# IONIQ6000/av1-base

Hardware: AMD Instinct MI355X
Metric: encoded frames/sec at CQ=30 (1080p intra-only) (higher is better)
Workload: dtype i32; 1 GPU; 1920x1080 60-frame all-key-frame synthclip v1 chunk per GPU, 10-bit 4:2:0, CQ=30 (base_q_idx 120), 32x32 blocks, all 13 intra candidates, 64x64 tiles, adaptive CDFs, CDEF on; frames_per_chunk=60, chunks_per_gpu=1, parallelism=chunk-per-gpu x1

## Files before the change

av1-base_amd/csrc/av1mi_dev.h:

```cpp
#ifndef AV1MI_DEV_H
#define AV1MI_DEV_H
#include <stdint.h>
#include <stddef.h>
#ifdef __HIPCC__
#define AV1MI_HD __host__ __device__
#else
#define AV1MI_HD
#endif

#define AV1MI_QM_4X4 0
#define AV1MI_QM_8X8 16
#define AV1MI_QM_16X16 80
#define AV1MI_QM_32X32 336
#define AV1MI_QM_PLANE 1360

struct Av1miQmEntry { uint32_t q, recip; };

struct Av1miChunkRecord {
  unsigned long long n_symbols;
  uint32_t max_tile_symbols;
  int overflow;
};
static_assert(sizeof(Av1miChunkRecord) == 16, "the frame offsets follow the head, 8-byte aligned");

// ... 197 lines not shown
    GLOBALMV = NEWMV + 6 * 3,
    REFMV = GLOBALMV + 2 * 3,
    DRL = REFMV + 6 * 3,
    SINGLE_REF = DRL + 3 * 3,
    INTER_TX1 = SINGLE_REF + 18 * 3,
    INTER_TX2 = INTER_TX1 + 2 * 17,
    INTER_TX3 = INTER_TX2 + 13,
    MV_JOINT = INTER_TX3 + 4 * 3,
    MV_COMP = MV_JOINT + 5,
    MVC_CLASS = 0, MVC_CLASS0_FP = 12, MVC_FP = 22, MVC_SIGN = 27, MVC_CLASS0_HP = 30, MVC_HP = 33, MVC_CLASS0 = 36, MVC_BITS = 39,
    MVC_SIZE = 69,
    TOTAL = MV_COMP + 2 * MVC_SIZE
  };
};

#endif
```

av1-base_amd/csrc/av1mi_host.cpp:

```cpp
#include <hip/hip_runtime.h>
#include <errno.h>
#include <math.h>
#include <stdarg.h>
#include <stdio.h>
#include <stdlib.h>
#include <string.h>
#include <unistd.h>

#include <algorithm>
#include <atomic>
#include <cstddef>
#include <mutex>
#include <string>
#include <thread>
#include <vector>

#include "../../include/av1mi.h"
#include "av1_tables.h"
#include "av1mi_dev.h"
#include "av1mi_launch.h"
#include "lr_fit_rule.h"
#include "wiener_fit_rule.h"
#include "deblock_pieces.h"
#include "aq_rule.h"
// ... 403 lines not shown
  unsigned long long *d_lrsse = nullptr;
  Av1miLrFit fit = {};
  uint8_t *d_fit = nullptr, *h_fit = nullptr;
  Av1miLrWfit wfit = {};
  uint8_t *d_wfit = nullptr, *h_wfit = nullptr;
  unsigned long long *d_cdef_err = nullptr;
  int8_t *d_cdef_idx = nullptr;
  uint8_t *d_cdef_sel = nullptr;
  unsigned long long *d_lf_err = nullptr;
  uint8_t *d_lf_sel = nullptr;
  uint8_t *h_lf = nullptr;
  uint8_t *h_out = nullptr;
  uint8_t *h_hdr = nullptr; uint16_t *h_cdf = nullptr; Av1miDevParams *h_params = nullptr;
  size_t hdr_bytes = 0;
  int cdf_qidx = -1;
  int params_on_device = 0;
  Av1miChunkRecord *h_record = nullptr; unsigned long long *h_sse = nullptr;
  size_t out_cap = 0, me64_bytes = 0, h_out_cap = 0;
  std::vector<std::pair<void *, bool>> owned;
};

template <class T>
hipError_t ws_alloc(Workspace &w, T *&p, size_t bytes, bool host = false) {
  for (auto b = w.owned.begin(); p && b != w.owned.end(); ++b)
    if (b->first == (void *)p) { (void)(b->second ? hipHostFree(p) : hipFree(p)); w.owned.erase(b); break; }
  void *v = nullptr;
  const hipError_t e = host ? hipHostMalloc(&v, bytes, hipHostMallocDefault) : hipMalloc(&v, bytes);
  if (e == hipSuccess) w.owned.emplace_back(v, host);
  p = (T *)v;
  return e;
// ... 64 lines not shown
                    w.scale == c->cap_scale && w.res.tile_sb == r.tile_sb;
  const int bps = p.bit_depth > 8 ? 2 : 1;
  const size_t frame_bytes = (size_t)r.cw * r.ch * 3 / 2 * bps;
  const size_t nsb = (size_t)r.sb_cols * r.sb_rows, ntile = (size_t)r.tile_cols * r.tile_rows, nb8 = (size_t)(r.cw / 8) * (r.ch / 8);
  if (!same) {
    free_workspace(c);
    const size_t nf = n_frames, slot = (size_t)tile_slot_bytes(r, c->cap_scale);
    for (void **b : { &w.d_src, &w.d_rec, &w.d_fin }) HIPCHK(c, ws_alloc(w, *b, nf * frame_bytes));
    HIPCHK(c, ws_alloc(w, w.d_levels, nf * nsb * AV1MI_SB_LEVELS * sizeof(int16_t)));
    HIPCHK(c, ws_alloc(w, w.d_blk, nf * nb8 * sizeof(Av1miBlkInfo)));
    HIPCHK(c, hipMemsetAsync(w.d_blk, 0, nf * nb8 * sizeof(Av1miBlkInfo), c->stream));
    HIPCHK(c, ws_alloc(w, w.d_slots, nf * ntile * slot * 2));
    w.out_cap = nf * (ntile * (slot + 4) + 256);
    HIPCHK(c, ws_alloc(w, w.d_out, w.out_cap));
    HIPCHK(c, ws_alloc(w, w.d_hdr, 256 + nf * 512));
    HIPCHK(c, ws_alloc(w, w.d_cdf, Av1miCdfLayout::TOTAL * sizeof(uint16_t)));
    HIPCHK(c, ws_alloc(w, w.d_params, AV1MI_AQ_SLOTS * sizeof(Av1miDevParams)));
    for (uint32_t **b : { &w.d_tile_bytes, &w.d_tile_off, &w.d_sym, &w.d_combos }) HIPCHK(c, ws_alloc(w, *b, nf * nsb * 4));
    HIPCHK(c, ws_alloc(w, w.d_streams, nf * ntile * (size_t)tile_stream_cap(r, c->cap_scale) * 4));
    for (uint32_t **b : { &w.d_frame_size, &w.d_payload }) HIPCHK(c, ws_alloc(w, *b, nf * 4));
    HIPCHK(c, ws_alloc(w, w.d_record, sizeof(Av1miChunkRecord) + (nf + 1) * 8));
    HIPCHK(c, ws_alloc(w, w.d_sse, nf * 3 * 8));
    {
      auto up = [](size_t n) { return (n + 255) & ~(size_t)255; };
      const size_t b_hdr = up(256 + nf * 512), b_cdf = up(Av1miCdfLayout::TOTAL * sizeof(uint16_t)), b_par = up(AV1MI_AQ_SLOTS * sizeof(Av1miDevParams)),
                   b_rec = up(sizeof(Av1miChunkRecord) + (nf + 1) * 8), b_sse = up(nf * 3 * 8);
      uint8_t *h = nullptr;
      HIPCHK(c, ws_alloc(w, h, b_hdr + b_cdf + b_par + b_rec + b_sse, true));
      w.h_hdr = h; h += b_hdr;
      w.h_cdf = reinterpret_cast<uint16_t *>(h); h += b_cdf;
      w.h_params = reinterpret_cast<Av1miDevParams *>(h); h += b_par;
      w.h_record = reinterpret_cast<Av1miChunkRecord *>(h); h += b_rec;
      w.h_sse = reinterpret_cast<unsigned long long *>(h);
    }
    HIPCHK(c, ws_alloc(w, w.d_me, nf * nb8 * 8));
    w.cap_frames = n_frames; w.scale = c->cap_scale;
  }
  const size_t nf = w.cap_frames;
  if (r.padded && !w.d_stage) HIPCHK(c, ws_alloc(w, w.d_stage, caller_bytes(r, nf)));
  if (p.partition_search && !w.d_part) HIPCHK(c, ws_alloc(w, w.d_part, nf * nsb * sizeof(uint32_t)));
// ... 463 lines not shown
  if (seq.size() > 256 || fh.size() > (size_t)P.hdr_slot_bytes || fhi.size() > (size_t)P.hdr_slot_bytes) { set_err(c, "internal: header larger than its slot"); return AV1MI_E_OVERFLOW; }
  std::vector<uint8_t> blob(seq.size() + (size_t)n_frames * P.hdr_slot_bytes, 0);
  memcpy(blob.data(), seq.data(), seq.size());
  for (uint32_t f = 0; f < n_frames; f++) {
    const bool inter = av1mi_frame_is_inter(P, (int)f);
    std::vector<uint8_t> &h = inter ? fhi : fh;
    if (r.p.film_grain && f) h = make_frame_header(r, nullptr, f, inter);
    memcpy(blob.data() + seq.size() + (size_t)f * P.hdr_slot_bytes, h.data(), h.size());
  }
  if (w.hdr_bytes != blob.size() || memcmp(w.h_hdr, blob.data(), blob.size())) {
    w.hdr_bytes = 0;
    memcpy(w.h_hdr, blob.data(), blob.size());
    HIPCHK(c, hipMemcpyAsync(w.d_hdr, w.h_hdr, blob.size(), hipMemcpyHostToDevice, s));
  }
  w.hdr_bytes = P.cdef_search || P.lf_search ? 0 : blob.size();
  if (w.cdf_qidx != r.qidx) {
    w.cdf_qidx = -1;
    const std::vector<uint16_t> cdf = make_cdf_blob(r.qidx);
    memcpy(w.h_cdf, cdf.data(), cdf.size() * 2);
    HIPCHK(c, hipMemcpyAsync(w.d_cdf, w.h_cdf, cdf.size() * 2, hipMemcpyHostToDevice, s));
    w.cdf_qidx = r.qidx;
  }
  {
    const int n_par = P.aq_map ? AV1MI_AQ_SLOTS : 1;
    std::vector<Av1miDevParams> par((size_t)n_par, P);
    for (int sl = 1; sl < n_par; sl++) {
      Av1miDevParams &Q = par[(size_t)sl];
      set_quant_steps(Q, quant_steps(av1mi_aq_slot_qindex(sl, r.qidx), P.bit_depth));
      if (P.qm_tab) Q.qm_tab = P.qm_tab + (size_t)sl * 2 * AV1MI_QM_PLANE;
    }
    const size_t bytes = (size_t)n_par * sizeof(P);
    if (w.params_on_device < n_par || memcmp(w.h_params, par.data(), bytes)) {
      w.params_on_device = 0;
      memcpy(w.h_params, par.data(), bytes);
      HIPCHK(c, hipMemcpyAsync(w.d_params, w.h_params, bytes, hipMemcpyHostToDevice, s));
      w.params_on_device = n_par;
// ... 264 lines not shown
```

av1-base_amd/csrc/entropy_kernel.hip:

```cpp
#include <hip/hip_runtime.h>
#include <cstdlib>
#include "av1mi_dev.h"
#include "av1mi_launch.h"

namespace {

typedef Av1miCdfLayout CL;

#define ENT_RESOLVED(fl6, fh6, ns) (0x80000000u | ((uint32_t)(fl6) << 14) | ((uint32_t)(fh6) << 4) | (uint32_t)(ns))
#define ENT_NARROW(slot, sym) (((uint32_t)(slot) << 2) | (uint32_t)(sym))
#define ENT_LITERAL(bit) ((bit) ? ENT_RESOLVED(256, 0, 0) : ENT_RESOLVED(512, 256, 1))
#define SLOTS_PER_COMBO 63
#define MAX_COMBOS 2

__shared__ uint16_t g_cdf_narrow[CL::INTRA_TOTAL - CL::COEFF_BASE + 64];
__shared__ uint16_t g_full_list[5 * 64];
__shared__ uint16_t g_cdf_inter[CL::TOTAL - CL::INTER_BASE + 64];
struct InterLds {
  int stk_row[10], stk_col[10], stk_w[10];
  uint8_t newmv[256];
};
__shared__ InterLds g_inter;
struct CC {
  enum {
    LEAD = CL::TX_SET1,
    TXSET = LEAD,
    TXB_SKIP = TXSET + 13 * 8,
    EOB = TXB_SKIP + 2 * 13 * 3,
    EOB_EXTRA = EOB + 2 * 12,
    DC_SIGN = EOB_EXTRA + 2 * 9 * 3,
    COEFF_BASE_EOB = DC_SIGN + 18,
    USE_WIENER = COEFF_BASE_EOB + 2 * 16, RESTORE_SW = USE_WIENER + 3, CFL_SIGN = RESTORE_SW + 4, CFL_ALPHA = CFL_SIGN + 9,
    DELTA_Q = CFL_ALPHA + 6 * 17,
    TOTAL = DELTA_Q + 5
  };
};
static_assert(CL::COEFF_BASE - CL::USE_WIENER == CC::TOTAL - CC::USE_WIENER, "the trailing tables are copied as one piece");
__shared__ uint16_t g_cdfw_full[CL::COEFF_BASE + 18];
__shared__ uint16_t g_cdfw_compact[CC::TOTAL + 18];
struct SymLds {
  alignas(16) int16_t lv[32 * 32];
  uint8_t left_lvl[3][16], left_dc[3][16];
};
__shared__ SymLds g_sym;
#define S (&g_sym)
template <int TSB>
struct TileLds {
  Av1miBlkInfo info[64 * TSB * TSB];
  uint8_t above_lvl[3][16 * TSB], above_dc[3][16 * TSB];
};
__shared__ TileLds<1> g_tile1;
__shared__ TileLds<2> g_tile2;
template <int TSB> struct TileSel;
template <> struct TileSel<1> { static __device__ __forceinline__ TileLds<1> &get() { return g_tile1; } };
template <> struct TileSel<2> { static __device__ __forceinline__ TileLds<2> &get() { return g_tile2; } };
#define TI (TileSel<TSB>::get())
#define TW (8 * TSB)

struct Sym {
  uint16_t *cdf;
  uint32_t *out;
  int pos;
  int cap;
  int combo0, combo1;
};

__device__ __forceinline__ int uni(int v) { return __builtin_amdgcn_readfirstlane(v); }
__device__ __forceinline__ int iabs(int v) { return v < 0 ? -v : v; }
__device__ __forceinline__ int imin(int a, int b) { return a < b ? a : b; }
__device__ __forceinline__ int imax(int a, int b) { return a > b ? a : b; }
__device__ __forceinline__ int floor_log2(unsigned v) { return 31 - __builtin_clz(v); }

__device__ __forceinline__ void emit1(Sym &y, int lane, uint32_t ent) {
  if (lane == 0 && y.pos < y.cap) y.out[y.pos] = ent;
  y.pos++;
}

template <int ARR = 0>
__device__ __forceinline__ void sym_wide(Sym &y, int lane, int adapt, int s, int off, int n) {
  s = uni(s); off = uni(off) - (ARR ? CL::INTER_BASE : 0); n = uni(n);
  const int v = ARR ? g_cdf_inter[off + (lane < 17 ? lane : 16)] : y.cdf[off + (lane < 17 ? lane : 16)];
  const uint32_t fl = s > 0 ? (uint32_t)__builtin_amdgcn_readlane(v, s - 1) : 32768u;
  const uint32_t fh = (uint32_t)__builtin_amdgcn_readlane(v, s);
  if (adapt) {
    const int cntr = __builtin_amdgcn_readlane(v, n);
    const int rate = 3 + (cntr > 15) + (cntr > 31) + (n > 3 ? 2 : 1);
    int nv = lane < s ? v + ((32768 - v) >> rate) : v - (v >> rate);
    nv = lane == n ? cntr + (cntr < 32) : nv;
    if (lane <= n) { if (ARR) g_cdf_inter[off + lane] = (uint16_t)nv; else y.cdf[off + lane] = (uint16_t)nv; }
  }
// ... 74 lines not shown
__device__ __forceinline__ void sym_coeffs(Sym &y, const int lane, const int adapt, const TileGeo &tg, int plane, int log2n, int x4,
                                           int y4, int eob, int ymode, int is_inter, const int16_t *lv_global) {
  const int idtx = ymode >> 8;
  ymode &= 255;
  const int ptype = plane > 0;
  const int txs = log2n - 2;
  const int w4 = (1 << log2n) >> 2;
  const int bwl = log2n > 5 ? 5 : log2n;
  const int n = 1 << bwl;
  const int max_x4 = plane ? tg.max_x4_c : tg.max_x4_y, max_y4 = plane ? tg.max_y4_c : tg.max_y4_y;
  const int aoff = (plane ? tg.tox >> 3 : tg.tox >> 2);
#define a_lvl (TI.above_lvl[plane] + aoff)
#define a_dc (TI.above_dc[plane] + aoff)
#define l_lvl S->left_lvl[plane]
#define l_dc S->left_dc[plane]
  typedef unsigned int u4 __attribute__((ext_vector_type(4)));
  u4 lv_pre[2];
  {
    const u4 *g128 = reinterpret_cast<const u4 *>(lv_global);
    const int last = n * n / 8 - 1;
    lv_pre[0] = g128[imin(lane, last)];
    lv_pre[1] = g128[imin(lane + 64, last)];
  }
  int nb_or = 0, dsum = 0;
  if (lane < w4) {
    if (x4 + lane < max_x4) { nb_or |= (a_lvl[x4 + lane] | a_dc[x4 + lane]) ? 1 : 0; int sg = a_dc[x4 + lane]; dsum += sg == 1 ? -1 : (sg == 2 ? 1 : 0); }
    if (y4 + lane < max_y4) { nb_or |= (l_lvl[y4 + lane] | l_dc[y4 + lane]) ? 2 : 0; int sg = l_dc[y4 + lane]; dsum += sg == 1 ? -1 : (sg == 2 ? 1 : 0); }
  }
  nb_or |= __builtin_amdgcn_update_dpp(0, nb_or, 0x128, 0xF, 0xF, false); dsum += __builtin_amdgcn_update_dpp(0, dsum, 0x128, 0xF, 0xF, false);
  nb_or |= __builtin_amdgcn_update_dpp(0, nb_or, 0x124, 0xF, 0xF, false); dsum += __builtin_amdgcn_update_dpp(0, dsum, 0x124, 0xF, 0xF, false);
  nb_or |= __builtin_amdgcn_update_dpp(0, nb_or, 0x122, 0xF, 0xF, false); dsum += __builtin_amdgcn_update_dpp(0, dsum, 0x122, 0xF, 0xF, false);
// ... 17 lines not shown
      const int tt = mode_txfm(ymode);
      if (log2n <= 3) sym_wide(y, lane, adapt, idtx ? 0 : txsym_set1(tt), FULL ? CL::TX_SET1 + ((log2n - 2) * 13 + ymode) * 8 : CC::TXSET + ymode * 8, 7);
      else sym_wide(y, lane, adapt, idtx ? 0 : txsym_set2(tt), FULL ? CL::TX_SET2 + ((log2n - 2) * 13 + ymode) * 6 : CC::TXSET + ymode * 6, 5);
    }
    {
      const int eob_pt = eob <= 2 ? eob : floor_log2((unsigned)(eob - 1)) + 2;
      const int base = eob_pt < 2 ? eob_pt : ((1 << (eob_pt - 2)) + 1);
      const int extra = eob - base;
      const int msz = 2 * bwl - 4;
      const int nsy = 5 + msz;
      const int eoff = CL::EOB16 + 4 * (msz * 6 + (msz * (msz - 1)) / 2);
      sym_wide(y, lane, adapt, eob_pt - 1, FULL ? eoff + (ptype * 2 + 0) * (nsy + 1) : CC::EOB + ptype * 12, nsy);
      if (eob_pt >= 3) {
        const int nbits = eob_pt - 2;
        sym_wide(y, lane, adapt, (extra >> (nbits - 1)) & 1, FULL ? CL::EOB_EXTRA + ((txs * 2 + ptype) * 9 + (eob_pt - 3)) * 3 : CC::EOB_EXTRA + (ptype * 9 + (eob_pt - 3)) * 3, 2);
        for (int i = 1; i < nbits; i++) emit1(y, lane, ENT_LITERAL((extra >> (nbits - 1 - i)) & 1));
      }
    }
#define scan(i_) scan_pos((i_), bwl)
    const int combo = txs * 2 + ptype;
    int slot0 = -1;
    if (adapt) {
      if (y.combo0 == combo) slot0 = 0;
      else if (y.combo0 < 0) { y.combo0 = combo; slot0 = 0; }
      else if (y.combo1 == combo) slot0 = SLOTS_PER_COMBO;
      else if (y.combo1 < 0) { y.combo1 = combo; slot0 = SLOTS_PER_COMBO; }
    }
    const int base_off0 = CL::COEFF_BASE + (txs * 2 + ptype) * 42 * 5;
    const int br_off0 = CL::COEFF_BR + ((txs > 3 ? 3 : txs) * 2 + ptype) * 21 * 5;
    int pos_nx = scan(imax(eob - 1 - lane, 0));
    {
// ... 16 lines not shown
        const int rc = row + col;
        cb = pos == 0 ? 0 : imin((mag + 1) >> 1, 4) + (rc < 2 ? rc : (rc < 4 ? 6 : 21));
        int mb = imin(a01, 15) + imin(a10, 15) + imin(a11, 15);
        mb = imin((mb + 1) >> 1, 6);
        cbr = pos == 0 ? mb : ((row < 2 && col < 2) ? mb + 7 : mb + 14);
        level = iabs((int)S->lv[pos]);
        const int nbr = level > 2 ? imin((level - 3) / 3 + 1, 4) : 0;
        cnt = (c != eob - 1) + nbr;
      }
      if (slot0 >= 0) {
        int total;
        const int off = wave_excl_scan(cnt, lane, &total);
        if (c >= 0 && y.pos + off + cnt <= y.cap) {
          uint32_t *o = y.out + y.pos + off;
          if (c != eob - 1) *o++ = ENT_NARROW(slot0 + cb, imin(level, 3));
          if (level > 2) {
            for (int idx = 0; idx < 4; idx++) {
              const int k3 = imin(level - 3 - idx * 3, 3);
              *o++ = ENT_NARROW(slot0 + 42 + cbr, k3);
              if (k3 < 3) break;
            }
          }
        }
        y.pos += total;
      } else if (FULL) {
        if constexpr (FULL) {
          int total;
          const int off = wave_excl_scan(cnt, lane, &total);
          if (c >= 0) {
            uint16_t *o = g_full_list + off;
            if (c != eob - 1) *o++ = (uint16_t)((cb << 2) | imin(level, 3));
            if (level > 2) {
              for (int idx = 0; idx < 4; idx++) {
                const int k3 = imin(level - 3 - idx * 3, 3);
                *o++ = (uint16_t)(((42 + cbr) << 2) | k3);
// ... 45 lines not shown
      const int fpos = fpos_nx;
      fpos_nx = scan(imin(c + 64, eob - 1));
      if (c < eob) v = S->lv[fpos];
      const int level = iabs(v);
      { int lsum; (void)wave_excl_scan(level, lane, &lsum); cul += lsum; }
      if (c0 == 0) {
        const int v0 = __builtin_amdgcn_readlane(v, 0);
        if (v0 != 0) {
          const int dctx = dsum < 0 ? 1 : (dsum > 0 ? 2 : 0);
          sym_wide(y, lane, adapt, v0 < 0, (FULL ? CL::DC_SIGN : CC::DC_SIGN) + (ptype * 3 + dctx) * 3, 2);
          dc_cat = v0 < 0 ? 1 : 2;
          const int l0 = iabs(v0);
          if (l0 > 14) {
            const unsigned g = (unsigned)(l0 - 15) + 1;
            const int len = floor_log2(g) + 1;
            for (int k = 0; k < len - 1; k++) emit1(y, lane, ENT_LITERAL(0));
            for (int k = len - 1; k >= 0; k--) emit1(y, lane, ENT_LITERAL((g >> k) & 1));
          }
        }
      }
      const bool mine = level != 0 && c != 0;
      const unsigned g = level > 14 ? (unsigned)(level - 15) + 1 : 0;
      const int glen = g ? floor_log2(g) + 1 : 0;
      const int cnt = mine ? 1 + (g ? 2 * glen - 1 : 0) : 0;
      int total;
      const int off = wave_excl_scan(cnt, lane, &total);
      if (mine && y.pos + off + cnt <= y.cap) {
        uint32_t *o = y.out + y.pos + off;
        *o++ = ENT_LITERAL(v < 0);
        if (g) {
          for (int k = 0; k < glen - 1; k++) *o++ = ENT_LITERAL(0);
          for (int k = glen - 1; k >= 0; k--) *o++ = ENT_LITERAL((g >> k) & 1);
// ... 161 lines not shown
template <bool FULL, bool INTER, int TSB>
__global__ void __launch_bounds__(64) symbolize_tile_kernel(Av1miDevParams P, const uint16_t *__restrict__ cdf_init,
                                                           const int16_t *__restrict__ levels, const Av1miBlkInfo *__restrict__ blk,
                                                           uint32_t *__restrict__ streams, uint32_t *__restrict__ stream_len,
                                                           uint32_t *__restrict__ tile_combos, const uint8_t *__restrict__ lr_choice,
                                                           int tile0 ,
                                                           int edge_grid ) {
  const int tiles_per_frame = P.tile_rows * P.tile_cols, sbs_per_frame = P.sb_rows * P.sb_cols;
  int gt = (int)blockIdx.x + tile0;
  if (edge_grid) { const int ne = av1mi_edge_tiles(P); gt = (tile0 / tiles_per_frame + (int)blockIdx.x / ne) * tiles_per_frame + av1mi_edge_tile(P, (int)blockIdx.x % ne); }
  const int f = gt / tiles_per_frame, tile = gt % tiles_per_frame;
  const int tr = tile / P.tile_cols, tc = tile % P.tile_cols;
  const int lane = threadIdx.x;
  if (av1mi_tile_is_regular(P, f, tr, tc, TSB) == FULL) return;
  if constexpr (FULL) {
    for (int i = lane; i < CL::COEFF_BASE; i += 64) g_cdfw_full[i] = cdf_init[i];
    if (lane < 18) g_cdfw_full[CL::COEFF_BASE + lane] = 0;
  } else {
    const int l2y = P.max_bs_log2 > 6 ? 6 : P.max_bs_log2, l2c = l2y - 1 > 5 ? 5 : l2y - 1;
    uint16_t *const w = g_cdfw_compact;
    for (int i = lane; i < CC::LEAD; i += 64) w[i] = cdf_init[i];
    for (int i = lane; i < 13 * 8; i += 64)
      w[CC::TXSET + i] = l2y <= 3 ? cdf_init[CL::TX_SET1 + (l2y - 2) * 13 * 8 + i] : ((l2y == 4 && i < 13 * 6) ? cdf_init[CL::TX_SET2 + (l2y - 2) * 13 * 6 + i] : (uint16_t)0);
    for (int i = lane; i < 2 * 39; i += 64) { const int p = i / 39, txs = (p ? l2c : l2y) - 2; w[CC::TXB_SKIP + i] = cdf_init[CL::TXB_SKIP + txs * 39 + i % 39]; }
    if (lane < 24) {
      const int p = lane / 12, k = lane % 12, bwl = (p ? l2c : l2y) > 5 ? 5 : (p ? l2c : l2y), msz = 2 * bwl - 4, nsy = 5 + msz;
      const int eoff = CL::EOB16 + 4 * (msz * 6 + (msz * (msz - 1)) / 2) + (p * 2 + 0) * (nsy + 1);
      w[CC::EOB + lane] = k <= nsy ? cdf_init[eoff + k] : (uint16_t)0;
    }
    if (lane < 2 * 27) { const int p = lane / 27, txs = (p ? l2c : l2y) - 2; w[CC::EOB_EXTRA + lane] = cdf_init[CL::EOB_EXTRA + (txs * 2 + p) * 27 + lane % 27]; }
    if (lane < 18) w[CC::DC_SIGN + lane] = cdf_init[CL::DC_SIGN + lane];
    if (lane < 2 * 16) { const int p = lane / 16, txs = (p ? l2c : l2y) - 2; w[CC::COEFF_BASE_EOB + lane] = cdf_init[CL::COEFF_BASE_EOB + (txs * 2 + p) * 16 + lane % 16]; }
    for (int i = lane; i < CC::TOTAL - CC::USE_WIENER; i += 64) w[CC::USE_WIENER + i] = cdf_init[CL::USE_WIENER + i];
    if (lane < 18) w[CC::TOTAL + lane] = 0;
  }
  if (FULL) {
    for (int i = lane; i < CL::INTRA_TOTAL - CL::COEFF_BASE; i += 64) g_cdf_narrow[i] = cdf_init[CL::COEFF_BASE + i];
    g_cdf_narrow[CL::INTRA_TOTAL - CL::COEFF_BASE + lane] = 0;
  }
  if (INTER) {
    for (int i = lane; i < CL::TOTAL - CL::INTER_BASE; i += 64) g_cdf_inter[i] = cdf_init[CL::INTER_BASE + i];
    g_cdf_inter[CL::TOTAL - CL::INTER_BASE + lane] = 0;
  }
  {
    const Av1miBlkInfo *finfo = blk + (size_t)f * P.b8_rows * P.b8_cols;
    for (int u = lane; u < 64 * TSB * TSB; u += 64) {
      const int r = tr * TW + u / TW, c = tc * TW + u % TW;
      Av1miBlkInfo bi = {};
      if (r < P.b8_rows && c < P.b8_cols) bi = finfo[(size_t)r * P.b8_cols + c];
      TI.info[u] = bi;
      if (INTER) g_inter.newmv[u] = 0;
    }
    for (int i = lane; i < 3 * 16 * TSB; i += 64) { (&TI.above_lvl[0][0])[i] = 0; (&TI.above_dc[0][0])[i] = 0; }
  }
  __syncthreads();
  Sym y;
  y.cdf = FULL ? g_cdfw_full : g_cdfw_compact;
  y.out = streams + (size_t)gt * P.stream_cap;
  y.pos = 0; y.cap = P.stream_cap;
  y.combo0 = -1; y.combo1 = -1;
  const int adapt = !P.disable_cdf_update;
  const int inter_frame = INTER;
  if (av1mi_frame_is_inter(P, f) != (int)INTER) return;
  int lr_prev = 0;
  int sgr_prev = 0;
// ... 23 lines not shown
    const int urows = imax((P.true_h + 32) / 64, 1), ucols = imax((P.true_w + 32) / 64, 1);
    if (sbr < urows && sbc < ucols) {
      const int nplanes = P.lr_chroma ? 3 : 1;
#pragma nounroll
      for (int pl = 0; pl < nplanes; pl++) {
        const int ch = uni(lr_choice[((size_t)f * nplanes + pl) * urows * ucols + sbr * ucols + sbc]);
        const bool wiener = ch <= 3 || (P.lr_wfit_code && ch == 23);
        if (P.enable_lr == 2) sym_wide(y, lane, adapt, ch == 0 ? 0 : (wiener ? 1 : 2), FULL ? CL::RESTORE_SW : CC::RESTORE_SW, 3);
        else sym_wide(y, lane, adapt, ch != 0, FULL ? CL::USE_WIENER : CC::USE_WIENER, 2);
        const int sh = 2 * pl;
        if (!wiener) {
          const uint32_t *fc = P.lr_fit_code ? P.lr_fit_code + (((size_t)f * 3 + pl) * urows * ucols + sbr * ucols + sbc) * 2 : nullptr;
          const int rf = (sgr_prev >> sh) & 3;
          const int len = fc ? uni((int)fc[1]) : P.sgr_code_len[rf][ch - 4];
          const unsigned long long bits = fc ? (unsigned long long)(uint32_t)uni((int)fc[0]) : P.sgr_code_bits[rf][ch - 4];
          for (int i = len - 1; i >= 0; i--) emit1(y, lane, ENT_LITERAL((int)((bits >> i) & 1)));
          if (!fc) sgr_prev = (sgr_prev & ~(3 << sh)) | ((ch - 3) << sh);
        } else if (ch && P.lr_wfit_code) {
          const uint32_t *wc = P.lr_wfit_code + (((size_t)f * 3 + pl) * urows * ucols + sbr * ucols + sbc) * 3;
          const int len = uni((int)wc[2]);
          const unsigned long long bits = (unsigned long long)(uint32_t)uni((int)wc[0]) | ((unsigned long long)(uint32_t)uni((int)wc[1]) << 32);
          for (int i = len - 1; i >= 0; i--) emit1(y, lane, ENT_LITERAL((int)((bits >> i) & 1)));
        } else if (ch) {
          const int rf = (lr_prev >> sh) & 3;
          const int len = pl ? P.lr_code_len_uv[rf][ch - 1] : P.lr_code_len[rf][ch - 1];
          const unsigned long long bits = pl ? P.lr_code_bits_uv[rf][ch - 1] : P.lr_code_bits[rf][ch - 1];
          for (int i = len - 1; i >= 0; i--) emit1(y, lane, ENT_LITERAL((int)((bits >> i) & 1)));
          lr_prev = (lr_prev & ~(3 << sh)) | (ch << sh);
        }
      }
    }
  }
#pragma nounroll
  for (int z = 0; z < 64; z++) {
    const int bx = (((z >> 0) & 1) | ((z >> 1) & 2) | ((z >> 2) & 4)) << 3;
    const int by = (((z >> 1) & 1) | ((z >> 2) & 2) | ((z >> 3) & 4)) << 3;
    if (tg.sb_y + by >= P.height || tg.sb_x + bx >= P.width) continue;
    const int b8x = bx >> 3, b8y = by >> 3;
    const int leaf = uni(INFO(b8x, b8y).bsl);
    if ((bx | by) & ((1 << leaf) - 1)) continue;
    const int top = imin(6, __builtin_ctz((unsigned)(bx | by | 64)));
#pragma nounroll
    for (int bsl = top; bsl >= leaf; bsl--) {
      const int n = 1 << bsl;
      const bool split = bsl > leaf;
      {
        const int half = n >> 1;
        const bool has_rows = tg.sb_y + by + half < P.height, has_cols = tg.sb_x + bx + half < P.width;
        const int above = by + toy > 0 && uni(INFO(b8x, b8y - 1).bsl) < bsl;
        const int left = bx + tox > 0 && uni(INFO(b8x - 1, b8y).bsl) < bsl;
        const int off = CL::PARTITION + ((bsl - 3) * 4 + left * 2 + above) * 11;
        if (has_rows && has_cols) {
          sym_wide(y, lane, adapt, split ? 3 : 0, off, bsl == 3 ? 4 : 10);
        } else if (has_cols) {
          int p = icdf_prob(y, off, 2) + icdf_prob(y, off, 3);
// ... 4 lines not shown
          if (bsl != 3) p += icdf_prob(y, off, 4) + icdf_prob(y, off, 5) + icdf_prob(y, off, 6) + icdf_prob(y, off, 8);
          sym_bool(y, lane, 1, (uint32_t)uni(p));
        }
      }
      if (split) continue;
      {
        const int ymode = uni(INFO(b8x, b8y).ymode), skip = uni(INFO(b8x, b8y).skip);
        const int eob0 = uni(INFO(b8x, b8y).eob[0]), eob1 = uni(INFO(b8x, b8y).eob[1]), eob2 = uni(INFO(b8x, b8y).eob[2]);
        const int avail_u = by + toy > 0, avail_l = bx + tox > 0;
        int sctx = 0;
        if (avail_u) sctx += uni(INFO(b8x, b8y - 1).skip);
        if (avail_l) sctx += uni(INFO(b8x - 1, b8y).skip);
        sym_wide(y, lane, adapt, skip, CL::SKIP + sctx * 3, 2);
        if (cdef_todo && !skip) {
          const int ci = uni(P.cdef_idx[(size_t)f * sbs_per_frame + sb]);
          for (int i = P.cdef_bits - 1; i >= 0; i--) sym_bool(y, lane, (ci >> i) & 1, 16384);
          cdef_todo = 0;
        }
        if (dq_todo) {
          dq_todo = 0;
          if (!(bsl == 6 && skip)) {
            const int qsb = uni(P.aq_map[(size_t)f * sbs_per_frame + sb]);
            const int r = (qsb - cur_q) / 4, a = iabs(r);
            sym_wide(y, lane, adapt, imin(a, 3), FULL ? CL::DELTA_Q : CC::DELTA_Q, 4);
            if (a >= 3) {
              const int nb = floor_log2((unsigned)(a - 1)), rest = a - 1 - (1 << nb);
              for (int i = 2; i >= 0; i--) sym_bool(y, lane, ((nb - 1) >> i) & 1, 16384);
              for (int i = nb - 1; i >= 0; i--) sym_bool(y, lane, (rest >> i) & 1, 16384);
            }
            if (a) sym_bool(y, lane, r < 0, 16384);
            cur_q = qsb;
          }
        }
        const int is_inter = inter_frame ? uni(INFO(b8x, b8y).is_inter) : 0;
        if (inter_frame) {
          const int a_intra = avail_u ? !uni(INFO(b8x, b8y - 1).is_inter) : 0;
          const int l_intra = avail_l ? !uni(INFO(b8x - 1, b8y).is_inter) : 0;
          int ictx;
          if (avail_u && avail_l) ictx = (l_intra && a_intra) ? 3 : ((l_intra || a_intra) ? 1 : 0);
          else if (avail_u || avail_l) ictx = 2 * (avail_u ? a_intra : l_intra);
          else ictx = 0;
          sym_wide<1>(y, lane, adapt, is_inter, CL::IS_INTER + ictx * 3, 2);
        }
        if (is_inter) {
          const int n_last = (avail_u ? uni(INFO(b8x, b8y - 1).is_inter) : 0) + (avail_l ? uni(INFO(b8x - 1, b8y).is_inter) : 0);
// ... 488 lines not shown
```

av1-base_amd/csrc/recon_kernel.hip:

```cpp
#include <hip/hip_runtime.h>
#include <type_traits>
#include "av1mi_dev.h"
#include "av1mi_launch.h"
#include "av1_tables.h"
#ifndef AV1MI_RECON_BIG
#define AV1MI_RECON_BIG 0
#endif
#ifndef AV1MI_RECON_PIX8
#define AV1MI_RECON_PIX8 0
#endif
#define MAXN (AV1MI_RECON_BIG ? 64 : 32)
#define AV1_TXFM_FN static __device__ __forceinline__
#define AV1_HALF_BTF_DEFINED
static __device__ __forceinline__ int32_t av1_half_btf(int32_t w0, int32_t a, int32_t w1, int32_t b) {
  return (__mul24(w0, a) + __mul24(w1, b) + 2048) >> 12;
}
#define AV1_HALF_BTF1_DEFINED
static __device__ __forceinline__ int32_t av1_half_btf1(int32_t w, int32_t a) { return (__mul24(w, a) + 2048) >> 12; }
#include "txfm_gen.h"
#include "fdct32_matrix.h"
#include "intra_pieces.h"
#include "quant_pieces.h"
#ifndef AV1MI_CHROMA_HANDOVER
#define AV1MI_CHROMA_HANDOVER 1
// ... 1278 lines not shown
}

__device__ __forceinline__ int leaf_bsl_at(const Av1miDevParams &P, int have_mask, uint32_t mask, int sb_x, int sb_y, int bx, int by) {
  return av1mi_leaf_bsl_at(P.width, P.height, P.min_bs_log2, P.max_bs_log2, have_mask, mask, sb_x, sb_y, bx, by);
}

template <typename PIX, bool INTER, int TSB, bool QM, bool SPLIT, bool EXT>
__device__ __forceinline__ void encode_superblock(const SbCtx &cx, const PIX *frame, PIX *rec_frame, int16_t *sb_levels,
                                                  Av1miBlkInfo *info, int b8_stride, const PIX *ref_frame,
                                                  const unsigned long long *me_best , int si,
                                                  int have_mask, uint32_t mask ) {
  const Av1miDevParams &P = *cx.P;
  constexpr int WL = SPLIT ? 1 : 0, WC = SPLIT ? 2 : 0;
  const int wv = SPLIT ? uniform_i((int)threadIdx.x >> 6) : 0;
#pragma nounroll
  for (int z = 0; z < 64; z++) {
    const int bx = (((z >> 0) & 1) | ((z >> 1) & 2) | ((z >> 2) & 4)) << 3;
    const int by = (((z >> 1) & 1) | ((z >> 2) & 2) | ((z >> 3) & 4)) << 3;
    if (cx.sb_y + by >= P.height || cx.sb_x + bx >= P.width) continue;
    const int bsl = leaf_bsl_at(P, have_mask, mask, cx.sb_x, cx.sb_y, bx, by);
    if (bsl == 0) continue;
    const int n = 1 << bsl;
    const int qi = si * 64 + z;
    int mode = 3 << 4;
    InterInfo ii;
    ii.ref = ref_frame; ii.is_inter = 0; ii.mv_row = ii.mv_col = 0; ii.sad_inter = 0;
    if constexpr (INTER) {
      const unsigned long long key = g_ws.key[(by >> 3) * 8 + (bx >> 3)];
      if (P.subpel) {
        ii.mv_row = (int16_t)(key >> 16); ii.mv_col = (int16_t)key;
        ii.sad_inter = (int)(key >> 36);
      } else {
        int dyv, dxv, cost;
        av1mi_me_key_decode(key, P.me_range, &dyv, &dxv, &cost);
        ii.mv_row = dyv * 8; ii.mv_col = dxv * 8;
        ii.sad_inter = cost - n * ((dxv < 0 ? -dxv : dxv) + (dyv < 0 ? -dyv : dyv));
// ... 311 lines not shown
```

Baseline: 21160 frames/s.

## Precompute compact CDF blob on host, vectorize LDS loads, batch literal emits, skip leaf z-steps

Moves the per-tile compact CDF table construction from the entropy kernel to the host, appending it to the uploaded CDF blob so each tile does a single vectorized 16-byte copy into shared memory. The full CDF and block-info loads also use 128-bit vector accesses. Serial per-bit literal emission loops, including the golomb, eob extra, LR, cdef and delta-q bits, become a single lane-parallel emit_bits. Coefficient range symbols are written unrolled, and both the recon and entropy z-order loops jump past the 8x8 positions covered by a larger leaf instead of visiting and rejecting them. Replacing sym_bool with literal entries for cdef and delta-q bits assumes the two encodings are equivalent.

```diff
diff --git a/av1-base_amd/csrc/av1mi_dev.h b/av1-base_amd/csrc/av1mi_dev.h
--- a/av1-base_amd/csrc/av1mi_dev.h
+++ b/av1-base_amd/csrc/av1mi_dev.h
@@ -235,4 +235,43 @@
   };
 };
 
+struct Av1miCdfCompact {
+  typedef Av1miCdfLayout CL;
+  enum {
+    LEAD = CL::TX_SET1,
+    TXSET = LEAD,
+    TXB_SKIP = TXSET + 13 * 8,
+    EOB = TXB_SKIP + 2 * 13 * 3,
+    EOB_EXTRA = EOB + 2 * 12,
+    DC_SIGN = EOB_EXTRA + 2 * 9 * 3,
+    COEFF_BASE_EOB = DC_SIGN + 18,
+    USE_WIENER = COEFF_BASE_EOB + 2 * 16, RESTORE_SW = USE_WIENER + 3, CFL_SIGN = RESTORE_SW + 4, CFL_ALPHA = CFL_SIGN + 9,
+    DELTA_Q = CFL_ALPHA + 6 * 17,
+    TOTAL = DELTA_Q + 5,
+    WORDS = (TOTAL + 18 + 7) & ~7,
+    AT = (CL::TOTAL + 7) & ~7,
+    BLOB_WORDS = AT + WORDS
+  };
+};
+static_assert(Av1miCdfLayout::COEFF_BASE - Av1miCdfLayout::USE_WIENER == Av1miCdfCompact::TOTAL - Av1miCdfCompact::USE_WIENER, "the trailing tables are copied as one piece");
+AV1MI_HD inline void av1mi_cdf_compact_build(const uint16_t *cdf, int max_bs_log2, uint16_t *w) {
+  typedef Av1miCdfLayout CL;
+  typedef Av1miCdfCompact CC;
+  const int l2y = max_bs_log2 > 6 ? 6 : max_bs_log2, l2c = l2y - 1 > 5 ? 5 : l2y - 1;
+  for (int i = 0; i < CC::WORDS; i++) w[i] = 0;
+  for (int i = 0; i < CC::LEAD; i++) w[i] = cdf[i];
+  if (l2y <= 3) for (int i = 0; i < 13 * 8; i++) w[CC::TXSET + i] = cdf[CL::TX_SET1 + (l2y - 2) * 13 * 8 + i];
+  else if (l2y == 4) for (int i = 0; i < 13 * 6; i++) w[CC::TXSET + i] = cdf[CL::TX_SET2 + (l2y - 2) * 13 * 6 + i];
+  for (int p = 0; p < 2; p++) {
+    const int l2 = p ? l2c : l2y, txs = l2 - 2, bwl = l2 > 5 ? 5 : l2, msz = 2 * bwl - 4, nsy = 5 + msz;
+    const int eoff = CL::EOB16 + 4 * (msz * 6 + (msz * (msz - 1)) / 2) + (p * 2 + 0) * (nsy + 1);
+    for (int k = 0; k < 39; k++) w[CC::TXB_SKIP + p * 39 + k] = cdf[CL::TXB_SKIP + txs * 39 + k];
+    for (int k = 0; k <= nsy; k++) w[CC::EOB + p * 12 + k] = cdf[eoff + k];
+    for (int k = 0; k < 27; k++) w[CC::EOB_EXTRA + p * 27 + k] = cdf[CL::EOB_EXTRA + (txs * 2 + p) * 27 + k];
+    for (int k = 0; k < 16; k++) w[CC::COEFF_BASE_EOB + p * 16 + k] = cdf[CL::COEFF_BASE_EOB + (txs * 2 + p) * 16 + k];
+  }
+  for (int i = 0; i < 18; i++) w[CC::DC_SIGN + i] = cdf[CL::DC_SIGN + i];
+  for (int i = 0; i < CC::TOTAL - CC::USE_WIENER; i++) w[CC::USE_WIENER + i] = cdf[CL::USE_WIENER + i];
+}
+
 #endif
diff --git a/av1-base_amd/csrc/av1mi_host.cpp b/av1-base_amd/csrc/av1mi_host.cpp
--- a/av1-base_amd/csrc/av1mi_host.cpp
+++ b/av1-base_amd/csrc/av1mi_host.cpp
@@ -441,6 +441,7 @@
   uint8_t *h_hdr = nullptr; uint16_t *h_cdf = nullptr; Av1miDevParams *h_params = nullptr;
   size_t hdr_bytes = 0;
   int cdf_qidx = -1;
+  int cdf_bs_log2 = -1;
   int params_on_device = 0;
   Av1miChunkRecord *h_record = nullptr; unsigned long long *h_sse = nullptr;
   size_t out_cap = 0, me64_bytes = 0, h_out_cap = 0;
@@ -535,7 +536,7 @@
     w.out_cap = nf * (ntile * (slot + 4) + 256);
     HIPCHK(c, ws_alloc(w, w.d_out, w.out_cap));
     HIPCHK(c, ws_alloc(w, w.d_hdr, 256 + nf * 512));
-    HIPCHK(c, ws_alloc(w, w.d_cdf, Av1miCdfLayout::TOTAL * sizeof(uint16_t)));
+    HIPCHK(c, ws_alloc(w, w.d_cdf, Av1miCdfCompact::BLOB_WORDS * sizeof(uint16_t)));
     HIPCHK(c, ws_alloc(w, w.d_params, AV1MI_AQ_SLOTS * sizeof(Av1miDevParams)));
     for (uint32_t **b : { &w.d_tile_bytes, &w.d_tile_off, &w.d_sym, &w.d_combos }) HIPCHK(c, ws_alloc(w, *b, nf * nsb * 4));
     HIPCHK(c, ws_alloc(w, w.d_streams, nf * ntile * (size_t)tile_stream_cap(r, c->cap_scale) * 4));
@@ -544,7 +545,7 @@
     HIPCHK(c, ws_alloc(w, w.d_sse, nf * 3 * 8));
     {
       auto up = [](size_t n) { return (n + 255) & ~(size_t)255; };
-      const size_t b_hdr = up(256 + nf * 512), b_cdf = up(Av1miCdfLayout::TOTAL * sizeof(uint16_t)), b_par = up(AV1MI_AQ_SLOTS * sizeof(Av1miDevParams)),
+      const size_t b_hdr = up(256 + nf * 512), b_cdf = up(Av1miCdfCompact::BLOB_WORDS * sizeof(uint16_t)), b_par = up(AV1MI_AQ_SLOTS * sizeof(Av1miDevParams)),
                    b_rec = up(sizeof(Av1miChunkRecord) + (nf + 1) * 8), b_sse = up(nf * 3 * 8);
       uint8_t *h = nullptr;
       HIPCHK(c, ws_alloc(w, h, b_hdr + b_cdf + b_par + b_rec + b_sse, true));
@@ -1038,12 +1039,14 @@
     HIPCHK(c, hipMemcpyAsync(w.d_hdr, w.h_hdr, blob.size(), hipMemcpyHostToDevice, s));
   }
   w.hdr_bytes = P.cdef_search || P.lf_search ? 0 : blob.size();
-  if (w.cdf_qidx != r.qidx) {
+  if (w.cdf_qidx != r.qidx || w.cdf_bs_log2 != P.max_bs_log2) {
     w.cdf_qidx = -1;
-    const std::vector<uint16_t> cdf = make_cdf_blob(r.qidx);
+    std::vector<uint16_t> cdf = make_cdf_blob(r.qidx);
+    cdf.resize(Av1miCdfCompact::BLOB_WORDS, 0);
+    av1mi_cdf_compact_build(cdf.data(), P.max_bs_log2, cdf.data() + Av1miCdfCompact::AT);
     memcpy(w.h_cdf, cdf.data(), cdf.size() * 2);
     HIPCHK(c, hipMemcpyAsync(w.d_cdf, w.h_cdf, cdf.size() * 2, hipMemcpyHostToDevice, s));
-    w.cdf_qidx = r.qidx;
+    w.cdf_qidx = r.qidx; w.cdf_bs_log2 = P.max_bs_log2;
   }
   {
     const int n_par = P.aq_map ? AV1MI_AQ_SLOTS : 1;
diff --git a/av1-base_amd/csrc/entropy_kernel.hip b/av1-base_amd/csrc/entropy_kernel.hip
--- a/av1-base_amd/csrc/entropy_kernel.hip
+++ b/av1-base_amd/csrc/entropy_kernel.hip
@@ -6,6 +6,7 @@
 namespace {
 
 typedef Av1miCdfLayout CL;
+typedef unsigned int u4 __attribute__((ext_vector_type(4)));
 
 #define ENT_RESOLVED(fl6, fh6, ns) (0x80000000u | ((uint32_t)(fl6) << 14) | ((uint32_t)(fh6) << 4) | (uint32_t)(ns))
 #define ENT_NARROW(slot, sym) (((uint32_t)(slot) << 2) | (uint32_t)(sym))
@@ -21,23 +22,9 @@
   uint8_t newmv[256];
 };
 __shared__ InterLds g_inter;
-struct CC {
-  enum {
-    LEAD = CL::TX_SET1,
-    TXSET = LEAD,
-    TXB_SKIP = TXSET + 13 * 8,
-    EOB = TXB_SKIP + 2 * 13 * 3,
-    EOB_EXTRA = EOB + 2 * 12,
-    DC_SIGN = EOB_EXTRA + 2 * 9 * 3,
-    COEFF_BASE_EOB = DC_SIGN + 18,
-    USE_WIENER = COEFF_BASE_EOB + 2 * 16, RESTORE_SW = USE_WIENER + 3, CFL_SIGN = RESTORE_SW + 4, CFL_ALPHA = CFL_SIGN + 9,
-    DELTA_Q = CFL_ALPHA + 6 * 17,
-    TOTAL = DELTA_Q + 5
-  };
-};
-static_assert(CL::COEFF_BASE - CL::USE_WIENER == CC::TOTAL - CC::USE_WIENER, "the trailing tables are copied as one piece");
-__shared__ uint16_t g_cdfw_full[CL::COEFF_BASE + 18];
-__shared__ uint16_t g_cdfw_compact[CC::TOTAL + 18];
+typedef Av1miCdfCompact CC;
+alignas(16) __shared__ uint16_t g_cdfw_full[(CL::COEFF_BASE + 18 + 7) & ~7];
+alignas(16) __shared__ uint16_t g_cdfw_compact[CC::WORDS];
 struct SymLds {
   alignas(16) int16_t lv[32 * 32];
   uint8_t left_lvl[3][16], left_dc[3][16];
@@ -46,7 +33,7 @@
 #define S (&g_sym)
 template <int TSB>
 struct TileLds {
-  Av1miBlkInfo info[64 * TSB * TSB];
+  alignas(16) Av1miBlkInfo info[64 * TSB * TSB];
   uint8_t above_lvl[3][16 * TSB], above_dc[3][16 * TSB];
 };
 __shared__ TileLds<1> g_tile1;
@@ -74,6 +61,14 @@
 __device__ __forceinline__ void emit1(Sym &y, int lane, uint32_t ent) {
   if (lane == 0 && y.pos < y.cap) y.out[y.pos] = ent;
   y.pos++;
+}
+__device__ __forceinline__ void emit_bits(Sym &y, int lane, unsigned long long bits, int len) {
+  if (lane < len && y.pos + lane < y.cap) y.out[y.pos + lane] = ENT_LITERAL((int)((bits >> ((len - 1 - lane) & 63)) & 1));
+  y.pos += len;
+}
+__device__ __forceinline__ void emit_bits(Sym &y, int lane, unsigned bits, int len) {
+  if (lane < len && y.pos + lane < y.cap) y.out[y.pos + lane] = ENT_LITERAL((int)((bits >> ((len - 1 - lane) & 31)) & 1));
+  y.pos += len;
 }
 
 template <int ARR = 0>
@@ -178,7 +173,6 @@
 #define a_dc (TI.above_dc[plane] + aoff)
 #define l_lvl S->left_lvl[plane]
 #define l_dc S->left_dc[plane]
-  typedef unsigned int u4 __attribute__((ext_vector_type(4)));
   u4 lv_pre[2];
   {
     const u4 *g128 = reinterpret_cast<const u4 *>(lv_global);
@@ -226,7 +220,7 @@
       if (eob_pt >= 3) {
         const int nbits = eob_pt - 2;
         sym_wide(y, lane, adapt, (extra >> (nbits - 1)) & 1, FULL ? CL::EOB_EXTRA + ((txs * 2 + ptype) * 9 + (eob_pt - 3)) * 3 : CC::EOB_EXTRA + (ptype * 9 + (eob_pt - 3)) * 3, 2);
-        for (int i = 1; i < nbits; i++) emit1(y, lane, ENT_LITERAL((extra >> (nbits - 1 - i)) & 1));
+        emit_bits(y, lane, (unsigned)extra, nbits - 1);
       }
     }
 #define scan(i_) scan_pos((i_), bwl)
@@ -273,11 +267,16 @@
         if (c >= 0 && y.pos + off + cnt <= y.cap) {
           uint32_t *o = y.out + y.pos + off;
           if (c != eob - 1) *o++ = ENT_NARROW(slot0 + cb, imin(level, 3));
-          if (level > 2) {
-            for (int idx = 0; idx < 4; idx++) {
-              const int k3 = imin(level - 3 - idx * 3, 3);
-              *o++ = ENT_NARROW(slot0 + 42 + cbr, k3);
-              if (k3 < 3) break;
+          const int nbr = cnt - (c != eob - 1);
+          const uint32_t br = ENT_NARROW(slot0 + 42 + cbr, 0);
+          if (nbr > 0) {
+            o[0] = br | (uint32_t)imin(level - 3, 3);
+            if (nbr > 1) {
+              o[1] = br | (uint32_t)imin(level - 6, 3);
+              if (nbr > 2) {
+                o[2] = br | (uint32_t)imin(level - 9, 3);
+                if (nbr > 3) o[3] = br | (uint32_t)imin(level - 12, 3);
+              }
             }
           }
         }
@@ -353,8 +352,7 @@
           if (l0 > 14) {
             const unsigned g = (unsigned)(l0 - 15) + 1;
             const int len = floor_log2(g) + 1;
-            for (int k = 0; k < len - 1; k++) emit1(y, lane, ENT_LITERAL(0));
-            for (int k = len - 1; k >= 0; k--) emit1(y, lane, ENT_LITERAL((g >> k) & 1));
+            emit_bits(y, lane, g, 2 * len - 1);
           }
         }
       }
@@ -546,25 +544,11 @@
   const int lane = threadIdx.x;
   if (av1mi_tile_is_regular(P, f, tr, tc, TSB) == FULL) return;
   if constexpr (FULL) {
-    for (int i = lane; i < CL::COEFF_BASE; i += 64) g_cdfw_full[i] = cdf_init[i];
+    for (int i = lane; i < CL::COEFF_BASE / 8; i += 64) reinterpret_cast<u4 *>(g_cdfw_full)[i] = reinterpret_cast<const u4 *>(cdf_init)[i];
+    if (lane < CL::COEFF_BASE % 8) g_cdfw_full[(CL::COEFF_BASE & ~7) + lane] = cdf_init[(CL::COEFF_BASE & ~7) + lane];
     if (lane < 18) g_cdfw_full[CL::COEFF_BASE + lane] = 0;
   } else {
-    const int l2y = P.max_bs_log2 > 6 ? 6 : P.max_bs_log2, l2c = l2y - 1 > 5 ? 5 : l2y - 1;
-    uint16_t *const w = g_cdfw_compact;
-    for (int i = lane; i < CC::LEAD; i += 64) w[i] = cdf_init[i];
-    for (int i = lane; i < 13 * 8; i += 64)
-      w[CC::TXSET + i] = l2y <= 3 ? cdf_init[CL::TX_SET1 + (l2y - 2) * 13 * 8 + i] : ((l2y == 4 && i < 13 * 6) ? cdf_init[CL::TX_SET2 + (l2y - 2) * 13 * 6 + i] : (uint16_t)0);
-    for (int i = lane; i < 2 * 39; i += 64) { const int p = i / 39, txs = (p ? l2c : l2y) - 2; w[CC::TXB_SKIP + i] = cdf_init[CL::TXB_SKIP + txs * 39 + i % 39]; }
-    if (lane < 24) {
-      const int p = lane / 12, k = lane % 12, bwl = (p ? l2c : l2y) > 5 ? 5 : (p ? l2c : l2y), msz = 2 * bwl - 4, nsy = 5 + msz;
-      const int eoff = CL::EOB16 + 4 * (msz * 6 + (msz * (msz - 1)) / 2) + (p * 2 + 0) * (nsy + 1);
-      w[CC::EOB + lane] = k <= nsy ? cdf_init[eoff + k] : (uint16_t)0;
-    }
-    if (lane < 2 * 27) { const int p = lane / 27, txs = (p ? l2c : l2y) - 2; w[CC::EOB_EXTRA + lane] = cdf_init[CL::EOB_EXTRA + (txs * 2 + p) * 27 + lane % 27]; }
-    if (lane < 18) w[CC::DC_SIGN + lane] = cdf_init[CL::DC_SIGN + lane];
-    if (lane < 2 * 16) { const int p = lane / 16, txs = (p ? l2c : l2y) - 2; w[CC::COEFF_BASE_EOB + lane] = cdf_init[CL::COEFF_BASE_EOB + (txs * 2 + p) * 16 + lane % 16]; }
-    for (int i = lane; i < CC::TOTAL - CC::USE_WIENER; i += 64) w[CC::USE_WIENER + i] = cdf_init[CL::USE_WIENER + i];
-    if (lane < 18) w[CC::TOTAL + lane] = 0;
+    for (int i = lane; i < CC::WORDS / 8; i += 64) reinterpret_cast<u4 *>(g_cdfw_compact)[i] = reinterpret_cast<const u4 *>(cdf_init + CC::AT)[i];
   }
   if (FULL) {
     for (int i = lane; i < CL::INTRA_TOTAL - CL::COEFF_BASE; i += 64) g_cdf_narrow[i] = cdf_init[CL::COEFF_BASE + i];
@@ -578,9 +562,9 @@
     const Av1miBlkInfo *finfo = blk + (size_t)f * P.b8_rows * P.b8_cols;
     for (int u = lane; u < 64 * TSB * TSB; u += 64) {
       const int r = tr * TW + u / TW, c = tc * TW + u % TW;
-      Av1miBlkInfo bi = {};
-      if (r < P.b8_rows && c < P.b8_cols) bi = finfo[(size_t)r * P.b8_cols + c];
-      TI.info[u] = bi;
+      u4 bi = {0u, 0u, 0u, 0u};
+      if (r < P.b8_rows && c < P.b8_cols) bi = *reinterpret_cast<const u4 *>(&finfo[(size_t)r * P.b8_cols + c]);
+      *reinterpret_cast<u4 *>(&TI.info[u]) = bi;
       if (INTER) g_inter.newmv[u] = 0;
     }
     for (int i = lane; i < 3 * 16 * TSB; i += 64) { (&TI.above_lvl[0][0])[i] = 0; (&TI.above_dc[0][0])[i] = 0; }
@@ -634,31 +618,33 @@
           const int rf = (sgr_prev >> sh) & 3;
           const int len = fc ? uni((int)fc[1]) : P.sgr_code_len[rf][ch - 4];
           const unsigned long long bits = fc ? (unsigned long long)(uint32_t)uni((int)fc[0]) : P.sgr_code_bits[rf][ch - 4];
-          for (int i = len - 1; i >= 0; i--) emit1(y, lane, ENT_LITERAL((int)((bits >> i) & 1)));
+          emit_bits(y, lane, bits, len);
           if (!fc) sgr_prev = (sgr_prev & ~(3 << sh)) | ((ch - 3) << sh);
         } else if (ch && P.lr_wfit_code) {
           const uint32_t *wc = P.lr_wfit_code + (((size_t)f * 3 + pl) * urows * ucols + sbr * ucols + sbc) * 3;
           const int len = uni((int)wc[2]);
           const unsigned long long bits = (unsigned long long)(uint32_t)uni((int)wc[0]) | ((unsigned long long)(uint32_t)uni((int)wc[1]) << 32);
-          for (int i = len - 1; i >= 0; i--) emit1(y, lane, ENT_LITERAL((int)((bits >> i) & 1)));
+          emit_bits(y, lane, bits, len);
         } else if (ch) {
           const int rf = (lr_prev >> sh) & 3;
           const int len = pl ? P.lr_code_len_uv[rf][ch - 1] : P.lr_code_len[rf][ch - 1];
           const unsigned long long bits = pl ? P.lr_code_bits_uv[rf][ch - 1] : P.lr_code_bits[rf][ch - 1];
-          for (int i = len - 1; i >= 0; i--) emit1(y, lane, ENT_LITERAL((int)((bits >> i) & 1)));
+          emit_bits(y, lane, bits, len);
           lr_prev = (lr_prev & ~(3 << sh)) | (ch << sh);
         }
       }
     }
   }
 #pragma nounroll
-  for (int z = 0; z < 64; z++) {
+  for (int z = 0, z_next; z < 64; z = z_next) {
+    z_next = z + 1;
     const int bx = (((z >> 0) & 1) | ((z >> 1) & 2) | ((z >> 2) & 4)) << 3;
     const int by = (((z >> 1) & 1) | ((z >> 2) & 2) | ((z >> 3) & 4)) << 3;
     if (tg.sb_y + by >= P.height || tg.sb_x + bx >= P.width) continue;
     const int b8x = bx >> 3, b8y = by >> 3;
     const int leaf = uni(INFO(b8x, b8y).bsl);
     if ((bx | by) & ((1 << leaf) - 1)) continue;
+    z_next = z + (1 << (2 * (leaf - 3)));
     const int top = imin(6, __builtin_ctz((unsigned)(bx | by | 64)));
 #pragma nounroll
     for (int bsl = top; bsl >= leaf; bsl--) {
@@ -693,7 +679,7 @@
         sym_wide(y, lane, adapt, skip, CL::SKIP + sctx * 3, 2);
         if (cdef_todo && !skip) {
           const int ci = uni(P.cdef_idx[(size_t)f * sbs_per_frame + sb]);
-          for (int i = P.cdef_bits - 1; i >= 0; i--) sym_bool(y, lane, (ci >> i) & 1, 16384);
+          emit_bits(y, lane, (unsigned)ci, P.cdef_bits);
           cdef_todo = 0;
         }
         if (dq_todo) {
@@ -704,10 +690,9 @@
             sym_wide(y, lane, adapt, imin(a, 3), FULL ? CL::DELTA_Q : CC::DELTA_Q, 4);
             if (a >= 3) {
               const int nb = floor_log2((unsigned)(a - 1)), rest = a - 1 - (1 << nb);
-              for (int i = 2; i >= 0; i--) sym_bool(y, lane, ((nb - 1) >> i) & 1, 16384);
-              for (int i = nb - 1; i >= 0; i--) sym_bool(y, lane, (rest >> i) & 1, 16384);
+              emit_bits(y, lane, (unsigned)(((nb - 1) << nb) | rest), 3 + nb);
             }
-            if (a) sym_bool(y, lane, r < 0, 16384);
+            if (a) emit_bits(y, lane, (unsigned)(r < 0), 1);
             cur_q = qsb;
           }
         }
diff --git a/av1-base_amd/csrc/recon_kernel.hip b/av1-base_amd/csrc/recon_kernel.hip
--- a/av1-base_amd/csrc/recon_kernel.hip
+++ b/av1-base_amd/csrc/recon_kernel.hip
@@ -1316,12 +1316,14 @@
   constexpr int WL = SPLIT ? 1 : 0, WC = SPLIT ? 2 : 0;
   const int wv = SPLIT ? uniform_i((int)threadIdx.x >> 6) : 0;
 #pragma nounroll
-  for (int z = 0; z < 64; z++) {
+  for (int z = 0, z_next; z < 64; z = z_next) {
+    z_next = z + 1;
     const int bx = (((z >> 0) & 1) | ((z >> 1) & 2) | ((z >> 2) & 4)) << 3;
     const int by = (((z >> 1) & 1) | ((z >> 2) & 2) | ((z >> 3) & 4)) << 3;
     if (cx.sb_y + by >= P.height || cx.sb_x + bx >= P.width) continue;
     const int bsl = leaf_bsl_at(P, have_mask, mask, cx.sb_x, cx.sb_y, bx, by);
     if (bsl == 0) continue;
+    z_next = z + (1 << (2 * (bsl - 3)));
     const int n = 1 << bsl;
     const int qi = si * 64 + z;
     int mode = 3 << 4;
```

New measurement: 23540 frames/s (median of 6 runs). +11.3%, better.
